# codeslake/RefVSR

Hardware: AMD Instinct MI355X
Metric: 4x SR frames/sec (270p->1080p, RefVSR_small_L1) (higher is better)
Workload: dtype f16; 1 GPU; config_RefVSR_small_L1 4x SR, 270x480 -> 1080x1920, frame_num=5, steady-state sliding window, n=1 (BASELINE configs[1]); synthetic clip seed 0, seeded random weights 1234; frames_per_rank=20, parallelism=frame-shard x1 (reset-aligned, no collective), window_cache=True, frame_ids=True, pipelined_calls=True, frames_per_call=4, headline_mode=frame groups, pipe_layout=pfm, full=False

## Files before the change

include/refvsr_hip.h:

```cpp
#ifndef REFVSR_HIP_H
#define REFVSR_HIP_H

#include <stddef.h>
#include <stdint.h>

#ifdef __cplusplus
extern "C" {
#endif

#define REFVSR_ABI_VERSION 15

int refvsr_abi_version(void);
int refvsr_max_maps(void);
const char* refvsr_last_error(void);
int refvsr_init(void);

int refvsr_num_cus(void);
int refvsr_stream_create_cu_range(int first_cu, int n_cus, void** stream);
int refvsr_stream_set_cu_budget(void* stream, int n_cus);
int refvsr_stream_destroy(void* stream);

enum { REFVSR_OUT_NHWC16 = 0, REFVSR_OUT_NHWC16_SHUFFLE2 = 1, REFVSR_OUT_PLANAR32 = 2 };

typedef struct RefvsrConv {
// ... 67 lines not shown
                     float* out, void* stream);
int refvsr_conv_hr_last(const void* src, int h, int w, const void* blob, float act_slope, const float* base_lr, int bh, int bw,
                        float* out, void* stream);
enum { REFVSR_RESULT_F32 = 0, REFVSR_RESULT_F16 = 1, REFVSR_RESULT_U8 = 2 };
int refvsr_conv_last_fmt(const void* src, int c, int h, int w, const void* blob, const float* base_lr, int bh, int bw,
                         void* out, int out_fmt, void* stream);
int refvsr_conv_hr_last_fmt(const void* src, int h, int w, const void* blob, float act_slope, const float* base_lr, int bh, int bw,
                            void* out, int out_fmt, void* stream);
int refvsr_convert_result(const float* src, size_t n, int out_fmt, void* out, void* stream);

int refvsr_conf_alpha(const float* conf_a, const float* conf_b, int h, int w, int up, const float* w0, const float* b0,
                      float slope0, const void* blob, int cout, float slope1, void* alpha, float* conf_max, void* stream);
int refvsr_conf_alpha_batch(const float* const* conf_a, const float* const* conf_b, int batch, int h, int w, int up, const float* w0,
                            const float* b0, float slope0, const void* blob, int cout, float slope1, void* const* alpha,
                            float* const* conf_max, void* stream);
int refvsr_conv32_supported(int c0, int c1);
int refvsr_conv32_blob_bytes(int c0, int c1);
int refvsr_conv32(const void* src0, int c0, const void* src1, int c1, int h, int w, const void* blob, float act_slope,
                  const void* mul, const void* res, float post_slope, void* out, void* stream);
int refvsr_conv48_supported(int c0, int c1);
int refvsr_conv48_blob_bytes(int c0, int c1);
int refvsr_conv48(const void* src0, int c0, const void* src1, int c1, int h, int w, const void* blob, float act_slope,
                  const void* mul, const void* res, float post_slope, void* out, void* stream);
int refvsr_conv_shuffle2_supported(int c);
int refvsr_conv_shuffle2_blob_bytes(int c);
int refvsr_conv_shuffle2(const void* src, int c, int h, int w, const void* blobs, float act_slope, void* out, void* stream);
int refvsr_conv_shuffle2_batch(const void* const* src, int batch, int c, int h, int w, const void* blobs, float act_slope,
                               void* const* out, void* stream);
int refvsr_conv24_f16w_blob_bytes(int c0, int c1);
int refvsr_conv32_f16w_blob_bytes(int c0, int c1);
int refvsr_conv_shuffle2_f16w_blob_bytes(int c);
int refvsr_conv24_f16w(const void* src0, int c0, const void* src1, int c1, int h, int w, const void* blob, float act_slope,
                       const void* mul, const void* res, float post_slope, void* out, void* stream);
int refvsr_conv24_batch_f16w(const void* const* src0, int c0, const void* const* src1, int c1, int batch, int h, int w, const void* blob,
                             float act_slope, const void* const* mul, const void* const* res, float post_slope, void* const* out,
                             void* stream);
int refvsr_conv32_f16w(const void* src0, int c0, const void* src1, int c1, int h, int w, const void* blob, float act_slope,
                       const void* mul, const void* res, float post_slope, void* out, void* stream);
int refvsr_conv_shuffle2_f16w(const void* src, int c, int h, int w, const void* blobs, float act_slope, void* out, void* stream);
int refvsr_conv_shuffle2_batch_f16w(const void* const* src, int batch, int c, int h, int w, const void* blobs, float act_slope,
                                    void* const* out, void* stream);
int refvsr_conf_alpha_f16w(const float* conf_a, const float* conf_b, int h, int w, int up, const float* w0, const float* b0,
                           float slope0, const void* blob, int cout, float slope1, void* alpha, float* conf_max, void* stream);
int refvsr_conf_alpha_batch_f16w(const float* const* conf_a, const float* const* conf_b, int batch, int h, int w, int up, const float* w0,
                                 const float* b0, float slope0, const void* blob, int cout, float slope1, void* const* alpha,
                                 float* const* conf_max, void* stream);
int refvsr_set_probe(void* buf, int iter);

int refvsr_conv_direct_f32(const float* src, int cin, int h, int w,
                           const float* wgt, const float* bias, int cout, int ksize, int stride, int pad,
                           float act_slope, void* out, int out_nhwc16, int out_c, void* stream);
int refvsr_conv1x1_f32(const float* src, int cin, int h, int w, const float* wgt, const float* bias, float act_slope,
                       float* out, void* stream);

int refvsr_pack_nhwc16(const float* src, int c, int h, int w, void* dst, int cs, void* stream);
int refvsr_pack_nhwc32(const float* src, int c, int h, int w, float* dst, int cs, void* stream);
int refvsr_unpack_nhwc16(const void* src, int h, int w, int cs, int c, float* dst, void* stream);

enum { REFVSR_RS_BICUBIC = 0, REFVSR_RS_BILINEAR = 1, REFVSR_RS_BILINEAR_AC = 2, REFVSR_RS_NEAREST = 3 };
int refvsr_resize(const float* src, int c, int h, int w, void* dst, int oh, int ow, int mode,
                  float src_scale_y, float src_scale_x, const float* mean, const float* std,
                  const float* chan_mul, int clamp01, int out_nhwc16, int out_c, void* stream);
int refvsr_avgpool2(const float* src, int c, int h, int w, float* dst, void* stream);
int refvsr_maxpool2(const float* src, int c, int h, int w, float* dst, void* stream);
int refvsr_avgpool_pyramid(const float* src, int c, int h, int w, float* const* dst, void* stream);
int refvsr_frame_prep(const float* lr, int h, int w, const float* ref, int hr, int wr, const float* wgt, const float* bias,
                      void* lr8, void* ref8, float* lr_n, float* ref_n, void* stream);
int refvsr_buffers_equal(const void* const* a, const void* const* b, int n_pairs, size_t n_bytes,
                         int32_t* flags, void* stream);
int refvsr_bytes_equal(const void* const* a, const void* const* b, int n_pairs, size_t n_bytes,
                       int32_t* flags, void* stream);
int refvsr_max2(const float* a, const float* b, float* out, size_t n, void* stream);

#define REFVSR_INGEST_MAX_FRAMES 16
enum { REFVSR_INGEST_PLANAR = 0, REFVSR_INGEST_HWC = 1 };
int refvsr_ingest_u8(const void* const* src, float* const* dst, int nframes, int h, int w, int layout, void* stream);
int refvsr_ingest_table(float* out);
int refvsr_ingest_max_frames(void);

#define REFVSR_SCORE_MAX_FRAMES 16
size_t refvsr_score_workspace_bytes(int nframes, int h, int w);
int refvsr_score_max_frames(void);
int refvsr_score_frames(const void* const* out, int out_fmt, const void* const* gt, int gt_fmt, int gt_layout, int nframes, int h, int w,
                        int win, void* workspace, size_t workspace_bytes, double* scores, void* stream);

int refvsr_score_frames_down(const void* const* out, int out_fmt, const void* const* gt, int gt_fmt, int gt_layout, int nframes, int h,
                             int w, int down, int win, void* workspace, size_t workspace_bytes, double* scores, void* stream);

#define REFVSR_SCORE_MAX_RECTS 8
size_t refvsr_score_regions_workspace_bytes(int nframes, int h, int w, int nrects);
int refvsr_score_max_rects(void);
int refvsr_score_regions(const void* const* out, int out_fmt, const void* const* gt, int gt_fmt, int gt_layout, int nframes, int h, int w,
                         const int* rects, int nrects, void* workspace, size_t workspace_bytes, double* sums, void* stream);

#define REFVSR_COLORMAP_MAX_MAPS 16
int refvsr_conf_colormap(const void* const* maps, int n, int h, int w, void* const* rgb, void* ws, size_t ws_bytes, void* stream);
size_t refvsr_conf_colormap_workspace_bytes(int n, int h, int w);
int refvsr_colormap_table(unsigned char* out768);

int refvsr_warp_nhwc16(const void* x, int hin, int win, int cs, const float* flow, int hf, int wf,
                       void* out, void* stream);
int refvsr_warp_nhwc16_up2(const void* x, int hin, int win, int cs, const float* flow_lr, int hl, int wl,
                           void* out, void* stream);
int refvsr_warp_planar(const float* x, int c, int hin, int win, const float* flow, int hf, int wf,
                       float* out, void* stream);
int refvsr_warp_nhwc16_batch(const void* const* x, int batch, int hin, int win, int cs, const float* const* flow, int hf, int wf,
// ... 48 lines not shown
```

refvsr_amd/engine.py:

```python
import collections
import itertools
import os

import torch

from . import ops
from .config import resolve_weight_precision
from .knobs import env_flag
from .packing import pack_conv
from .weights import VGG_MEAN, VGG_STD, round16

_uid = itertools.count()


def _timed_event(stream):
    e = torch.cuda.Event(enable_timing=True)
    e.record(stream)
    return e


def _flow_pairs(fr, restart):
    t = len(fr)
    ctr = t // 2
    need = [(fr[i], fr[i + 1]) for i in range(ctr, t - 1)] + [(fr[ctr + 1], fr[ctr])]
# ... 124 lines not shown
        reslist('feat_decoder_BWFW', 4)
        for br in ('backward_resblocks', 'forward_resblocks'):
            cin = sd['Network.' + br + '.main.0.weight'].shape[1]
            if cin == C + 3:
                mf(br + '.main.0', [3, C])
            else:
                assert cin == 2 * C + 3
                mf(br + '.main.0', [3, C, C])
                cw = self.conv[br + '.main.0']
                cw.cpads = [cw.cpads[0] + cw.cpads[1], cw.cpads[2]]
            for i in range(self.nb):
                mf('%s.main.2.%d.conv1' % (br, i), [C])
                mf('%s.main.2.%d.conv2' % (br, i), [C])
        mf('fusion_UP', [C, C])
        mf('upsample1.upsample_conv', [C], shuffle=True)
        if config.scale == 4:
            mf('upsample2.upsample_conv', [C], shuffle=True)
        mf('conv_hr', [C])
        mf('conv_last', [C])


class Engine(object):

    def __init__(self, config, weights):
        if config.scale not in (2, 4):
            raise NotImplementedError('SR scale must be 2 or 4 (configs/config_RefVSR_*.py: "SR scale (2 | 4)")')
        self.cfg = config
        self.W = weights
        self.C = config.mid_channels
        self.nb = config.num_blocks
        self.ks = config.matching_ksize
        self.hd = bool(config.flag_HD_in)
        self.vgg7 = self.hd or config.scale != 4
        self.cache = bool(getattr(config, 'cache_windows', True))
        self.match_row_splits = 1
        self.match_margin = float(getattr(config, 'match_exact_margin', ops.MATCH_EXACT_MARGIN))
        self.chain_calls = bool(getattr(config, 'chain_calls', not env_flag('REFVSR_NO_CHAIN_CALLS')))
        self.fuse_resblocks = (bool(getattr(config, 'fuse_resblocks', True)) and ops.resblock_fits(self.C)
                               and not env_flag('REFVSR_NO_FUSE'))
        self.rb24 = not env_flag('REFVSR_NO_RB24')
        self.rb48 = (bool(getattr(config, 'fuse_resblocks', True)) and not env_flag('REFVSR_NO_FUSE')
                     and not env_flag('REFVSR_NO_RB48'))
        self.rb48_max_pixels = int(os.environ.get('REFVSR_RB48_MAX_PIXELS', str(540 * 960)))
        self.rb48_multimap = not env_flag('REFVSR_NO_RB48_MULTIMAP')
        self.spynet_mt1_pixels = int(os.environ.get('REFVSR_SPYNET_MT1_PIXELS', str(72 * 120)))
        self.bw_head_blocks = min(self.nb, max(-1, int(getattr(config, 'bw_head_blocks', None) if getattr(config, 'bw_head_blocks', None) is not None
                                                         else os.environ.get('REFVSR_BW_HEAD_BLOCKS', '12'))))
        self.warp_up2 = not env_flag('REFVSR_NO_WARP_UP2')
        self.fuse_head = not env_flag('REFVSR_NO_FUSE_HEAD')
        self.fuse_tail = self.fuse_head and (env_flag('REFVSR_FUSE_TAIL') or bool(getattr(config, 'fuse_tail', False)))
        self.fuse_conf = not env_flag('REFVSR_NO_FUSE_CONF')
        self.map1x1 = not env_flag('REFVSR_NO_MAP1X1')
        self.legacy_prep = env_flag('REFVSR_LEGACY_PREP')
        self.last_flagged = None
        self.spynet_batch = not env_flag('REFVSR_NO_SPYNET_BATCH')
        self.overlap = bool(getattr(config, 'overlap_streams', True)) and not env_flag('REFVSR_NO_OVERLAP')
        self._side = None
        self.pipelined = bool(getattr(config, 'pipelined', False))
        self._zero_maps = {}
        self.result_dtype = str(getattr(config, 'result_dtype', None) or 'float32').replace('torch.', '')
        ops.result_format(self.result_dtype)
        self._pipe = None
        self._layout_default = None
        self.pipe_depth = max(1, int(getattr(config, 'pipe_depth', None) or os.environ.get('REFVSR_PIPE_DEPTH') or 3))
        self._inflight = collections.deque()
        self.stream_events = None
        self.kernel_events = None
        self.chain_events = None
        self.reset_state()

    def reset_state(self):
        self.fw_feat = None
        self.fw_flow = None
        self.fw_feat_up = None
        self.fw_conf = None
        self.frame_itr_num = 0
        self.max_frame_itr_num = self.cfg.reset_branch
        self.prev_window = []
        self.flow_cache = {}
        self.id_cache = {}
        self.ctx_pinned = {}
        self.ctx_strict = False
        self._fw_up_wait = None

    def set_pipelined(self, on=True):
        self.pipelined = bool(on)

    def export_state(self):
        if self.fw_feat is None:
            return None
        self._await_fw_up(self.fw_feat_up)
        st = dict(feat=ops.unpack_nhwc16(self.fw_feat, self.C), flow=self.fw_flow, feat_up=ops.unpack_nhwc16(self.fw_feat_up, self.C),
                  conf=self.fw_conf, frame_itr_num=self.frame_itr_num)
        kf = getattr(self, 'keyframe_idx', None)
        if kf is not None:
            st['keyframe_idx'] = [int(k) for k in kf]
        return st

    def import_state(self, st):
        cs = (self.C + 7) // 8 * 8
        self.fw_feat = ops.pack_nhwc16(st['feat'].contiguous(), cs)
        self.fw_flow = st['flow'].contiguous()
        self.fw_feat_up = ops.pack_nhwc16(st['feat_up'].contiguous(), cs)
        self.fw_conf = st['conf'].contiguous()
        self.frame_itr_num = int(st['frame_itr_num'])
        if st.get('keyframe_idx') is not None and hasattr(self, 'keyframe_idx'):
# ... 334 lines not shown
                x = ops.conv(cw if cw is not None else self.cw(p + '%d.conv' % j), x, act=0.0, batch=B)
            flow = ops.conv(self.cw(p + '4.conv'), x, planar_out=True, res_planar=fup, batch=B)
        h_up, w_up = flow.shape[2:]
        cm = [float(w) / float(w_up), float(h) / float(h_up)]
        outs = [ops.resize(flow[b0:b0 + 2].reshape(-1, h_up, w_up), (h, w), ops.RS_BILINEAR, chan_mul=cm * min(2, B - b0))
                for b0 in range(0, B, 2)]
        out = outs[0].view(-1, 2, h, w) if len(outs) == 1 else torch.cat([o_.view(-1, 2, h, w) for o_ in outs], 0)
        ev = None
        if share:
            ev = torch.cuda.Event()
            ev.record()
            for st in share:
                out.record_stream(st)
        for i, (a, b) in enumerate(todo):
            self.flow_cache[(a.uid, b.uid)] = (out[i], ev)

    def frame_prep(self, fr):
        if self.hd or self.legacy_prep:
            return None
        return ops.frame_prep(fr.lr, fr.ref, *self.W.raw['feature_match.sub_mean'])

    def feature_match(self, fr, prep=None):
        R = self.W.raw
        h, w = fr.lr.shape[1:]

        fe = 'feature_match.feature_extract.'

        def extract(x):
            x = ops.conv(self.cw(fe + '0'), x, act=0.0)
            if not self.vgg7:
                x = ops.conv(self.cw(fe + '2'), x, act=0.0)
                if self.map1x1:
                    return ops.conv1x1_f32(x, *R[fe + 'map64.0'], act=0.2)
                return ops.conv(self.cw(fe + 'map64.0'), x, act=0.2, planar_out=True)
            x = ops.conv(self.cw(fe + '2'), x, act=0.0, planar_out=True)
            x = ops.pack_nhwc32(ops.maxpool2(x))
            x = ops.conv(self.cw(fe + '5'), x, act=0.0)
            if self.map1x1:
                return ops.conv1x1_f32(x, *R[fe + 'map128.0'], act=0.2)
            return ops.conv(self.cw(fe + 'map128.0'), x, act=0.2, planar_out=True)
        if prep is None:
            prep = self.frame_prep(fr)
        if prep is not None:
            lr_n, ref_n = prep[2], prep[3]
        else:
            lr_n = ops.conv_direct(fr.lr, *R['feature_match.sub_mean'])
            ref_n = ops.conv_direct(fr.ref, *R['feature_match.sub_mean'])
            if self.hd:
                f = 1.0 / (self.cfg.scale // 2)
                oh, ow = int(h * f), int(w * f)
                lr_n = ops.resize(lr_n, (oh, ow), ops.RS_NEAREST, (1.0 / f, 1.0 / f))
                ref_n = ops.resize(ref_n, (oh, ow), ops.RS_NEAREST, (1.0 / f, 1.0 / f))
            lr_n, ref_n = ops.pack_nhwc32(lr_n, 4), ops.pack_nhwc32(ops.avgpool2(ref_n), 4)
        lr_f = extract(lr_n)
        ref_f = extract(ref_n)
        ops.set_match_patches_kernel(0 if self.legacy_prep else 1)
        if self.legacy_prep:
            lr_rows, inv_lr, lr_lo = ops.match_patches(lr_f, ops.hip.MATCH_COLBLOCK, want_lo=True)
        else:
            (lr_rows, inv_lr), lr_lo = ops.match_patches(lr_f, ops.hip.MATCH_COLBLOCK), None
        ref_rows, inv_ref, ref_lo = ops.match_patches(ref_f, ops.hip.MATCH_ROWCHUNK, want_lo=True)
        n_lr = lr_f.shape[1] * lr_f.shape[2]
        n_ref = ref_f.shape[1] * ref_f.shape[2]
        if self.kernel_events is not None:
            e0, e1 = torch.cuda.Event(enable_timing=True), torch.cuda.Event(enable_timing=True)
            e0.record()
        cand, cand_val = ops.match_top2(ref_rows, n_ref, lr_rows, n_lr, self.match_row_splits)
        if self.kernel_events is not None:
            e1.record()
            self.kernel_events.append((e0, e1))
        conf, idx, self.last_flagged = ops.match_refine(lr_f, ref_f, inv_lr, inv_ref, cand, cand_val, self.match_margin, (lr_rows, lr_lo),
                                                        (ref_rows, ref_lo))
        conf = conf.view(1, lr_f.shape[1], lr_f.shape[2])
        grid = (lr_f.shape[1], lr_f.shape[2])
        if grid[0] != h:
            conf = ops.bicubic_scale(conf, float(h) / grid[0], clamp01=True)
        return conf, idx, grid

    def aligned_conv(self, feats, query, rgb8, prefix, ks):
        def enc(z8):
            e = ops.conv(self.cw(prefix + '.conv1.0'), z8, act=0.2)
            t = ops.conv(self.cw(prefix + '.conv1.2.conv1'), e, act=0.2)
            return ops.conv(self.cw(prefix + '.conv1.2.conv2'), t, res=e, post=0.2)
        q = enc(ops.bicubic_scale(query, 2, clamp01=False, nhwc16_out=True))
        r = enc(rgb8)
        a = ops.conv(self.cw(prefix + '.p_conv.0'), r, q, stride=ks, act=0.2)
        t = ops.conv(self.cw(prefix + '.p_conv.2.conv1'), a, act=0.2)
        a = ops.conv(self.cw(prefix + '.p_conv.2.conv2'), t, res=a, post=0.2)
        affine = ops.conv(self.cw(prefix + '.p_conv.4'), a, planar_out=True, add_const=1.0, clamp=(-3.0, 3.0))
        return ops.aligned_sample(feats, affine, ks)

    def _ref_encoders(self, fr, ref8=None):
        if ref8 is None:
            ref8 = ops.pack_nhwc16(fr.ref, 8)
        x = ops.conv(self.cw('ref_encoder1.0.0'), ref8, act=0.2)
        x = ops.conv(self.cw('ref_encoder1.1.0'), x, act=0.2)
        ref_feat = self.res_list(x, 'res1', 4)
        x = ops.conv(self.cw('ref_encoder2.0.0'), ref_feat, stride=2, act=0.2)
        x = ops.conv(self.cw('ref_encoder2.1.0'), x, act=0.2)
        return ref_feat, self.res_list(x, 'res2', 4)

    def prepare_frame(self, fr):
        if fr.conf is not None:
            return
        if self.ctx_strict:
            raise RuntimeError('a window needs a per-frame context that was neither prepared ahead nor imported (strict mode)')
        h, w = fr.lr.shape[1:]
        prep = self.frame_prep(fr)
# ... 797 lines not shown
```

refvsr_amd/hip.py:

```python
import ctypes as C
import os

_HERE = os.path.dirname(os.path.abspath(__file__))
LIB_PATH = os.path.join(_HERE, 'librefvsr_hip.so')

OUT_NHWC16, OUT_NHWC16_SHUFFLE2, OUT_PLANAR32 = 0, 1, 2
RS_BICUBIC, RS_BILINEAR, RS_BILINEAR_AC, RS_NEAREST = 0, 1, 2, 3
RESULT_F32, RESULT_F16, RESULT_U8 = 0, 1, 2
INGEST_PLANAR, INGEST_HWC = 0, 1
MATCH_KP, MATCH_ROWCHUNK, MATCH_COLBLOCK = 152, 256, 512
ABI_VERSION = 15
MAX_MAPS = 4
INGEST_MAX_FRAMES = 16
SCORE_MAX_FRAMES = 16
SCORE_MAX_RECTS = 8
COLORMAP_MAX_MAPS = 16
RESBLOCK24_BLOB_BYTES = 43264
RESBLOCK24_F16W_BLOB_BYTES = 28928
RESBLOCK48_BLOB_BYTES = 172544


class RefvsrConv(C.Structure):
    _fields_ = [
        ('src0', C.c_void_p), ('c0', C.c_int),
# ... 74 lines not shown
    'refvsr_conv_hr_last_fmt': [_P, _I, _I, _P, _F, _P, _I, _I, _P, _I, _P],
    'refvsr_convert_result': [_P, _Z, _I, _P, _P],
    'refvsr_conf_alpha': [_P, _P, _I, _I, _I, _P, _P, _F, _P, _I, _F, _P, _P, _P],
    'refvsr_spynet_level_input_batch': [_P, _P, _I, _P, _I, _I, _P, _P, _P],
    'refvsr_resblock24_chain_batch': [_P, _I, _I, _I, _I, _P, _Z, _F, _P, _P, _P, _P],
    'refvsr_resblock48_chain_batch': [_P, _I, _I, _I, _I, _P, _Z, _F, _P, _P, _P, _P],
    'refvsr_conv24_batch': [_P, _I, _P, _I, _I, _I, _I, _P, _F, _P, _P, _F, _P, _P],
    'refvsr_conv_shuffle2_batch': [_P, _I, _I, _I, _I, _P, _F, _P, _P],
    'refvsr_conf_alpha_batch': [_P, _P, _I, _I, _I, _I, _P, _P, _F, _P, _I, _F, _P, _P, _P],
    'refvsr_warp_nhwc16_batch': [_P, _I, _I, _I, _I, _P, _I, _I, _P, _P],
    'refvsr_warp_nhwc16_up2_batch': [_P, _I, _I, _I, _I, _P, _I, _I, _P, _P],
    'refvsr_warp_planar_batch': [_P, _I, _I, _I, _I, _P, _I, _I, _P, _P],
    'refvsr_match_patches': [_P, _I, _I, _P, _P, _P, _P],
    'refvsr_match_top2': [_P, _I, _P, _I, _I, _P, _P, _P],
    'refvsr_match_refine': [_P, _I, _I, _P, _I, _I, _P, _P, _P, _P, _I, _F, _P, _P, _P, _P],
    'refvsr_match_exact': [_P, _I, _I, _P, _I, _I, _P, _P, _P, _P, _P, _P, _P, _P, _P, _P, _P],
    'refvsr_match_naive': [_P, _I, _I, _P, _I, _I, _P, _P, _P],
    'refvsr_block_gather_nhwc16': [_P, _I, _I, _I, _P, _I, _I, _I, _P, _P],
    'refvsr_block_gather_rgb': [_P, _I, _I, _P, _I, _I, _I, _P, _P, _P],
    'refvsr_aligned_sample': [_P, _I, _I, _I, _I, _P, _P, _P],
    'refvsr_dcn_sample': [_P, _I, _I, _I, _P, _I, _P, _P],
    'refvsr_tsa_weight': [_P, _P, _P, _I, _I, _I, _P, _P],
    'refvsr_pool3s2_nhwc16': [_P, _I, _I, _I, _P, _I, _I, _I, _P],
    'refvsr_up2_bilinear_nhwc16': [_P, _I, _I, _I, _F, _P, _P],
    'refvsr_tsa_blend': [_P, _P, _P, _Z, _P, _P],
    'refvsr_resblock24_f16w_blob_bytes': [],
    'refvsr_conv24_f16w_blob_bytes': [_I, _I],
    'refvsr_conv32_f16w_blob_bytes': [_I, _I],
    'refvsr_conv_shuffle2_f16w_blob_bytes': [_I],
    'refvsr_resblock24_chain_f16w': [_P, _I, _I, _I, _P, _Z, _F, _P, _P, _P, _P],
    'refvsr_resblock24_chain_batch_f16w': [_P, _I, _I, _I, _I, _P, _Z, _F, _P, _P, _P, _P],
    'refvsr_conv24_f16w': [_P, _I, _P, _I, _I, _I, _P, _F, _P, _P, _F, _P, _P],
    'refvsr_conv24_batch_f16w': [_P, _I, _P, _I, _I, _I, _I, _P, _F, _P, _P, _F, _P, _P],
    'refvsr_conv32_f16w': [_P, _I, _P, _I, _I, _I, _P, _F, _P, _P, _F, _P, _P],
    'refvsr_conv_shuffle2_f16w': [_P, _I, _I, _I, _P, _F, _P, _P],
    'refvsr_conv_shuffle2_batch_f16w': [_P, _I, _I, _I, _I, _P, _F, _P, _P],
    'refvsr_conf_alpha_f16w': [_P, _P, _I, _I, _I, _P, _P, _F, _P, _I, _F, _P, _P, _P],
    'refvsr_conf_alpha_batch_f16w': [_P, _P, _I, _I, _I, _I, _P, _P, _F, _P, _I, _F, _P, _P, _P],
    'refvsr_ingest_u8': [_P, _P, _I, _I, _I, _I, _P],
    'refvsr_ingest_table': [_P],
    'refvsr_ingest_max_frames': [],
    'refvsr_bytes_equal': [_P, _P, _I, _Z, _P, _P],
    'refvsr_score_frames': [_P, _I, _P, _I, _I, _I, _I, _I, _I, _P, _Z, _P, _P],
    'refvsr_score_max_frames': [],
    'refvsr_score_frames_down': [_P, _I, _P, _I, _I, _I, _I, _I, _I, _I, _P, _Z, _P, _P],
    'refvsr_score_regions': [_P, _I, _P, _I, _I, _I, _I, _I, _P, _I, _P, _Z, _P, _P],
    'refvsr_score_max_rects': [],
    'refvsr_set_match_patches_kernel': [_I],
    'refvsr_match_lo_rows': [_P, _I, _I, _P, _P, _P, _P],
    'refvsr_avgpool_pyramid': [_P, _I, _I, _I, _P, _P],
    'refvsr_frame_prep': [_P, _I, _I, _P, _I, _I, _P, _P, _P, _P, _P, _P, _P],
    'refvsr_conf_colormap': [_P, _I, _I, _I, _P, _P, _Z, _P],
    'refvsr_colormap_table': [_P],
}
_SPECIAL = {'refvsr_abi_version': (C.c_int, []), 'refvsr_last_error': (C.c_char_p, []),
            'refvsr_score_workspace_bytes': (C.c_size_t, [_I, _I, _I]),
            'refvsr_score_regions_workspace_bytes': (C.c_size_t, [_I, _I, _I, _I]),
            'refvsr_conf_colormap_workspace_bytes': (C.c_size_t, [_I, _I, _I])}
EXPORTS = tuple(sorted(list(SIGNATURES) + list(_SPECIAL)))

_lib = None


def lib():
    global _lib
    if _lib is None:
        if not os.path.exists(LIB_PATH):
            raise RuntimeError(
                'refvsr_amd: %s not found -- the HIP extension is required (no CPU fallback). '
                'Build it with `make -C refvsr_amd/csrc` or `python -c "import __graft_entry__ as g; g.build()"`.'
                % LIB_PATH)
        h = C.CDLL(LIB_PATH)
        for name, args in SIGNATURES.items():
            fn = getattr(h, name)
            fn.argtypes = args
            fn.restype = C.c_int
        for name, (res, args) in _SPECIAL.items():
            fn = getattr(h, name)
            fn.argtypes = args
            fn.restype = res
        if h.refvsr_abi_version() != ABI_VERSION:
            raise RuntimeError('refvsr_amd: ABI mismatch (library %d, binding %d)' % (h.refvsr_abi_version(), ABI_VERSION))
        if h.refvsr_max_maps() != MAX_MAPS:
            raise RuntimeError('refvsr_amd: REFVSR_MAX_MAPS mismatch (library %d, binding %d)' % (h.refvsr_max_maps(), MAX_MAPS))
        if h.refvsr_ingest_max_frames() != INGEST_MAX_FRAMES:
            raise RuntimeError('refvsr_amd: REFVSR_INGEST_MAX_FRAMES mismatch (library %d, binding %d)'
                               % (h.refvsr_ingest_max_frames(), INGEST_MAX_FRAMES))
        if h.refvsr_score_max_frames() != SCORE_MAX_FRAMES:
            raise RuntimeError('refvsr_amd: REFVSR_SCORE_MAX_FRAMES mismatch (library %d, binding %d)'
                               % (h.refvsr_score_max_frames(), SCORE_MAX_FRAMES))
        if h.refvsr_score_max_rects() != SCORE_MAX_RECTS:
            raise RuntimeError('refvsr_amd: REFVSR_SCORE_MAX_RECTS mismatch (library %d, binding %d)'
                               % (h.refvsr_score_max_rects(), SCORE_MAX_RECTS))
        _lib = h
    return _lib


def check(rc, what):
    if rc != 0:
        msg = lib().refvsr_last_error()
        raise RuntimeError('refvsr_hip.%s failed (rc=%d): %s' % (what, rc, msg.decode() if msg else '?'))
```

refvsr_amd/ops.py:

```python
import ctypes as C
import math
import os

import torch

from . import hip
from .knobs import env_flag
from .hip import (OUT_NHWC16, OUT_NHWC16_SHUFFLE2, OUT_PLANAR32, RS_BICUBIC, RS_BILINEAR,
                  RS_BILINEAR_AC, RS_NEAREST)


_STREAM = None


def _stream():
    if _STREAM is not None:
        return _STREAM
    return C.c_void_p(torch.cuda.current_stream().cuda_stream)


class on_stream(object):

    def __init__(self, stream):
        self.stream = stream
# ... 408 lines not shown
    hip.check(hip.lib().refvsr_convert_result(_ptr(x), x.numel(), fmt, _ptr(out), _stream()), 'convert_result')
    return out


def conv_last(blob, src, base_lr, result_dtype=None):
    _nhwc(src)
    _planar(base_lr, 3)
    h, w, c = src.shape
    bh, bw = base_lr.shape[1:]
    dt, fmt = result_format(result_dtype)
    out = torch.empty((3, h, w), dtype=dt, device=src.device)
    hip.check(hip.lib().refvsr_conv_last_fmt(_ptr(src), c, h, w, _ptr(blob), _ptr(base_lr), bh, bw, _ptr(out), fmt, _stream()), 'conv_last')
    return out


def conv_hr_last(blob, src, base_lr, act=0.1, result_dtype=None):
    _nhwc(src)
    _planar(base_lr, 3)
    h, w, c = src.shape
    assert c == 24 and blob.numel() == hip.RESBLOCK24_BLOB_BYTES
    bh, bw = base_lr.shape[1:]
    dt, fmt = result_format(result_dtype)
    out = torch.empty((3, h, w), dtype=dt, device=src.device)
    hip.check(hip.lib().refvsr_conv_hr_last_fmt(_ptr(src), h, w, _ptr(blob), act, _ptr(base_lr), bh, bw, _ptr(out), fmt, _stream()), 'conv_hr_last')
    return out


def conv_last_ok(c, h, w):
    return bool(hip.lib().refvsr_conv_last_supported(int(c))) and h * w * c * 2 < 2 ** 31


def conf_alpha_ok(cw):
    return cw.blob24 is not None and cw.cpads == [16] and cw.cout in (24, 48) and not cw.shuffle


def pack_nhwc16(x, cs=None):
    _planar(x)
    c, h, w = x.shape
    cs = cs or (c + 7) // 8 * 8
    out = torch.empty((h, w, cs), dtype=torch.float16, device=x.device)
    hip.check(hip.lib().refvsr_pack_nhwc16(_ptr(x), c, h, w, _ptr(out), cs, _stream()), 'pack_nhwc16')
    return out


def conv1x1_f32(x, w, b, act=0.2):
    assert x.is_cuda and x.dtype == torch.float32 and x.dim() == 3 and x.is_contiguous()
    h, w_, cin = x.shape
    assert tuple(w.shape) == (16, cin) and w.dtype == torch.float32 and w.is_contiguous() and tuple(b.shape) == (16,)
    out = torch.empty((16, h, w_), dtype=torch.float32, device=x.device)
    hip.check(hip.lib().refvsr_conv1x1_f32(_ptr(x), cin, h, w_, _ptr(w), _ptr(b), float(act), _ptr(out), _stream()), 'conv1x1_f32')
    return out


def pack_nhwc32(x, cs=None):
    _planar(x)
    c, h, w = x.shape
    cs = cs or (c + 3) // 4 * 4
    out = torch.empty((h, w, cs), dtype=torch.float32, device=x.device)
    hip.check(hip.lib().refvsr_pack_nhwc32(_ptr(x), c, h, w, _ptr(out), cs, _stream()), 'pack_nhwc32')
    return out


def unpack_nhwc16(x, c=None):
    _nhwc(x)
    h, w, cs = x.shape
    c = c or cs
    out = torch.empty((c, h, w), dtype=torch.float32, device=x.device)
    hip.check(hip.lib().refvsr_unpack_nhwc16(_ptr(x), h, w, cs, c, _ptr(out), _stream()), 'unpack_nhwc16')
    return out


def resize(x, out_hw, mode, src_scale=None, mean=None, std=None, chan_mul=None, clamp01=False, nhwc16_out=False):
    _planar(x)
    c, h, w = x.shape
    oh, ow = out_hw
    if src_scale is None:
        src_scale = (float(h) / float(oh), float(w) / float(ow))
    if nhwc16_out:
        out = torch.empty((oh, ow, 8), dtype=torch.float16, device=x.device)
    else:
        out = torch.empty((c, oh, ow), dtype=torch.float32, device=x.device)
    hip.check(hip.lib().refvsr_resize(_ptr(x), c, h, w, _ptr(out), oh, ow, mode, src_scale[0], src_scale[1],
                                      _farr(mean), _farr(std), _farr(chan_mul), int(clamp01), int(nhwc16_out),
                                      8 if nhwc16_out else 0, _stream()), 'resize')
    return out


def bicubic_scale(x, factor, clamp01=True, nhwc16_out=False):
    c, h, w = x.shape
    oh, ow = int(math.floor(h * factor)), int(math.floor(w * factor))
    s = 1.0 / factor
    return resize(x, (oh, ow), RS_BICUBIC, (s, s), clamp01=clamp01, nhwc16_out=nhwc16_out)


def flow_up2(flow):
    c, h, w = flow.shape
    return resize(flow, (2 * h, 2 * w), RS_BILINEAR_AC, (0.0, 0.0), chan_mul=[2.0] * c)


def avgpool2(x):
    _planar(x)
    c, h, w = x.shape
    out = torch.empty((c, h // 2, w // 2), dtype=torch.float32, device=x.device)
    hip.check(hip.lib().refvsr_avgpool2(_ptr(x), c, h, w, _ptr(out), _stream()), 'avgpool2')
    return out

# ... 594 lines not shown
```

Baseline: 233.3 frames/s.

## Fuse VGG feature-match head (conv0, conv2, 1x1 map) into one multi-map kernel

Adds a single HIP kernel that runs the feature-match VGG head in one pass: first 3x3 conv (3->64), second 3x3 conv (64->64) via f32 MFMA with a ring-buffered LDS weight pipeline, and the 64->16 1x1 map. It covers both LR and reference maps in one launch and is used by default when the 1x1 map path is active. This removes the intermediate 64-channel feature maps in global memory and several kernel launches. In exchange it adds heavy LDS use per block (low occupancy) and recomputes a halo for conv0 in each tile.

Result: no change. 235.3 frames/s (median of 6 runs) (+0.9%).

```diff
diff --git a/include/refvsr_hip.h b/include/refvsr_hip.h
--- a/include/refvsr_hip.h
+++ b/include/refvsr_hip.h
@@ -143,6 +143,9 @@
                            float act_slope, void* out, int out_nhwc16, int out_c, void* stream);
 int refvsr_conv1x1_f32(const float* src, int cin, int h, int w, const float* wgt, const float* bias, float act_slope,
                        float* out, void* stream);
+int refvsr_vgg_head(const void* const* src, const int* h, const int* w, int n, const void* wpack0, const float* bias0,
+                    const void* wpack2, const float* bias2, const float* wmap, const float* bmap, float map_slope,
+                    void* const* out, void* stream);
 
 int refvsr_pack_nhwc16(const float* src, int c, int h, int w, void* dst, int cs, void* stream);
 int refvsr_pack_nhwc32(const float* src, int c, int h, int w, float* dst, int cs, void* stream);
diff --git a/refvsr_amd/csrc/vgg_head.hip b/refvsr_amd/csrc/vgg_head.hip
--- /dev/null
+++ b/refvsr_amd/csrc/vgg_head.hip
@@ -0,0 +1,325 @@
+#include "common.h"
+
+#define VH_NW 8
+#define VH_TH 8
+#define VH_TW 32
+#define VH_XH (VH_TH + 4)
+#define VH_XW (VH_TW + 4)
+#define VH_FH (VH_TH + 2)
+#define VH_FW (VH_TW + 2)
+#define VH_FPIX (VH_FH * VH_FW)
+#define VH_PS 17
+#define VH_S0 3
+#define VH_S2 36
+#define VH_CH 4
+#define VH_NCHUNK (VH_S2 / VH_CH)
+#define VH_NS 3
+#define VH_SLOT (VH_CH * 4 * 1024)
+#define VH_PPW (VH_CH * 4 / VH_NW)
+#define VH_YS 65
+
+#define VH_OFF_TAB2 0
+#define VH_OFF_TAB0 (VH_S2 * 16)
+#define VH_OFF_RING 640
+#define VH_OFF_X (VH_OFF_RING + VH_NS * VH_SLOT)
+#define VH_OFF_F (VH_OFF_X + VH_XH * VH_XW * 16)
+#define VH_LDS (VH_OFF_F + VH_FPIX * VH_PS * 16)
+
+static_assert(VH_OFF_TAB0 + VH_S0 * 16 <= VH_OFF_RING, "tables");
+static_assert(VH_S2 % VH_CH == 0 && VH_PPW * VH_NW == VH_CH * 4 && VH_CH == 4, "the ring loop is unrolled for 4 full K-steps per chunk");
+static_assert(VH_TH * VH_TW * VH_YS * 4 <= VH_FPIX * VH_PS * 16 && 64 * 16 * 4 <= VH_XH * VH_XW * 16, "epilogue regions");
+static_assert(VH_LDS <= 160 * 1024, "LDS");
+
+struct VHArgs {
+    const unsigned char* src[REFVSR_MAX_MAPS];
+    float* out[REFVSR_MAX_MAPS];
+    int h[REFVSR_MAX_MAPS], w[REFVSR_MAX_MAPS], tiles_x[REFVSR_MAX_MAPS];
+    int t_end[REFVSR_MAX_MAPS];
+    int n;
+    const unsigned char* w0; const float* b0;
+    const unsigned char* w2; const float* b2;
+    const float* wm; const float* bm;
+    float slope;
+};
+
+__global__ __launch_bounds__(VH_NW * 64) void vgg_head_kernel(VHArgs p) {
+    extern __shared__ __attribute__((aligned(16))) unsigned char smem[];
+    int* tab2 = reinterpret_cast<int*>(smem + VH_OFF_TAB2);
+    int* tab0 = reinterpret_cast<int*>(smem + VH_OFF_TAB0);
+    unsigned char* ring = smem + VH_OFF_RING;
+    unsigned char* xt = smem + VH_OFF_X;
+    unsigned char* ft = smem + VH_OFF_F;
+
+    int tl = blockIdx.x;
+    const unsigned char* src = p.src[0];
+    float* out = p.out[0];
+    int h = p.h[0], w = p.w[0], tiles_x = p.tiles_x[0], t0 = 0;
+#pragma unroll
+    for (int m = 1; m < REFVSR_MAX_MAPS; ++m)
+        if (m < p.n && tl >= p.t_end[m - 1]) { src = p.src[m]; out = p.out[m]; h = p.h[m]; w = p.w[m]; tiles_x = p.tiles_x[m]; t0 = p.t_end[m - 1]; }
+    tl -= t0;
+    asm volatile("" :: "s"(src), "s"(out), "s"(h), "s"(w), "s"(tiles_x), "s"(tl), "s"(p.w0), "s"(p.b0), "s"(p.w2), "s"(p.b2),
+                 "s"(p.wm), "s"(p.bm), "s"(p.slope));
+    const int tyi = tl / tiles_x;
+    const int ty0 = tyi * VH_TH;
+    const int tx0 = (tl - tyi * tiles_x) * VH_TW;
+
+    const int tid = threadIdx.x;
+    const int lane = tid & 63;
+    const int wave = tid >> 6;
+    const int q = lane >> 4;
+    const int lp = rv_pix16(lane & 15);
+
+    const int wv = __builtin_amdgcn_readfirstlane(wave);
+    const unsigned char* gw = p.w2 + lane * 16;
+    auto issue = [&](const int c, const int slot) {
+#pragma unroll
+        for (int j = 0; j < VH_PPW; ++j) {
+            const int pc = wv + j * VH_NW;
+            const int s = c * VH_CH + (pc >> 2), m = pc & 3;
+            __builtin_amdgcn_global_load_lds((const __attribute__((address_space(1))) void*)(gw + (((m >> 1) * VH_S2 + s) * 2 + (m & 1)) * 1024),
+                                             (__attribute__((address_space(3))) void*)(ring + slot * VH_SLOT + pc * 1024), 16, 0, 0);
+        }
+    };
+    int slot_w = 0;
+    for (int c = 0; c < VH_NS - 1; ++c) { issue(c, slot_w); ++slot_w; }
+
+    if (tid < VH_S2 * 4) {
+        const int tap = tid >> 4, cg = tid & 15;
+        const int ty = tap / 3, tx = tap - ty * 3;
+        tab2[rv_kslot(ty, tx, cg, 3, 16)] = ((ty * VH_FW + tx) * VH_PS + cg) * 16;
+    } else if (tid < VH_S2 * 4 + VH_S0 * 4) {
+        const int g = tid - VH_S2 * 4;
+        if (g < 9) {
+            const int ty = g / 3, tx = g - ty * 3;
+            tab0[rv_kslot(ty, tx, 0, 3, 1)] = (ty * VH_XW + tx) * 16;
+        } else {
+            tab0[rv_kpad_slot(g - 9, 3, 1)] = 16;
+        }
+    }
+    if (tid < VH_XH * VH_XW) {
+        const int r = tid / VH_XW, c = tid - r * VH_XW;
+        const int iy = ty0 - 2 + r, ix = tx0 - 2 + c;
+        const bool ok = (unsigned)iy < (unsigned)h && (unsigned)ix < (unsigned)w;
+        const size_t pix = (size_t)min(max(iy, 0), h - 1) * w + min(max(ix, 0), w - 1);
+        uint4 v = *reinterpret_cast<const uint4*>(src + pix * 16);
+        const unsigned keep = ok ? 0xffffffffu : 0u;
+        v.x &= keep; v.y &= keep; v.z &= keep; v.w &= keep;
+        *reinterpret_cast<uint4*>(xt + tid * 16) = v;
+    }
+    uint4 a0w[VH_S0][4];
+    float4 b0r[4];
+#pragma unroll
+    for (int s = 0; s < VH_S0; ++s)
+#pragma unroll
+        for (int m = 0; m < 4; ++m)
+            a0w[s][m] = *reinterpret_cast<const uint4*>(p.w0 + ((((m >> 1) * VH_S0 + s) * 2 + (m & 1)) * 64 + lane) * 16);
+#pragma unroll
+    for (int m = 0; m < 4; ++m) b0r[m] = *reinterpret_cast<const float4*>(p.b0 + m * 16 + q * 4);
+    __syncthreads();
+
+    for (int g = wave; g * 16 < VH_FPIX; g += VH_NW) {
+        const int pp = g * 16 + lp;
+        const int pc = min(pp, VH_FPIX - 1);
+        const int r = pc / VH_FW, c = pc - r * VH_FW;
+        const unsigned char* xb = xt + (r * VH_XW + c) * 16;
+        f32x4 acc0[4];
+#pragma unroll
+        for (int m = 0; m < 4; ++m) acc0[m] = (f32x4){0.f, 0.f, 0.f, 0.f};
+#pragma unroll
+        for (int s = 0; s < VH_S0; ++s) {
+            const f32x4 bv = *reinterpret_cast<const f32x4*>(xb + tab0[s * 4 + q]);
+#pragma unroll
+            for (int m = 0; m < 4; ++m) {
+                const f32x4 av = *reinterpret_cast<const f32x4*>(&a0w[s][m]);
+#pragma unroll
+                for (int j = 0; j < 4; ++j) acc0[m] = __builtin_amdgcn_mfma_f32_16x16x4f32(av[j], bv[j], acc0[m], 0, 0, 0);
+            }
+        }
+        const int iy = ty0 - 1 + r, ix = tx0 - 1 + c;
+        const bool inside = (unsigned)iy < (unsigned)h && (unsigned)ix < (unsigned)w;
+        if (pp < VH_FPIX) {
+#pragma unroll
+            for (int m = 0; m < 4; ++m) {
+                float y[4];
+                const float4 bv = b0r[m];
+                y[0] = acc0[m][0] + bv.x; y[1] = acc0[m][1] + bv.y; y[2] = acc0[m][2] + bv.z; y[3] = acc0[m][3] + bv.w;
+#pragma unroll
+                for (int i = 0; i < 4; ++i) y[i] = inside ? rv_lrelu(y[i], 0.0f) : 0.0f;
+                *reinterpret_cast<f32x4*>(ft + (pp * VH_PS + m * 4 + q) * 16) = (f32x4){y[0], y[1], y[2], y[3]};
+            }
+        }
+    }
+
+    f32x4 acc[4][2];
+#pragma unroll
+    for (int m = 0; m < 4; ++m)
+#pragma unroll
+        for (int t = 0; t < 2; ++t) acc[m][t] = (f32x4){0.f, 0.f, 0.f, 0.f};
+    {
+        const unsigned lds_tab = (unsigned)(size_t)(__attribute__((address_space(3))) unsigned char*)reinterpret_cast<unsigned char*>(tab2);
+        const unsigned lds_ring = (unsigned)(size_t)(__attribute__((address_space(3))) unsigned char*)ring;
+        const unsigned lds_ft = (unsigned)(size_t)(__attribute__((address_space(3))) unsigned char*)ft;
+        unsigned pbaddr[2];
+#pragma unroll
+        for (int t = 0; t < 2; ++t) pbaddr[t] = lds_ft + (unsigned)(((wave * VH_FW + t * 16 + lp) * VH_PS) * 16);
+        typedef unsigned u32x4 __attribute__((ext_vector_type(4)));
+        auto tie = [](uint4& r) {
+            u32x4 t = {r.x, r.y, r.z, r.w};
+            asm volatile("" : "+v"(t));
+            r = make_uint4(t[0], t[1], t[2], t[3]);
+        };
+        auto wait_set = [&](uint4 (&a)[4], uint4 (&b)[2]) {
+            asm volatile("s_waitcnt lgkmcnt(6)" ::: "memory");
+#pragma unroll
+            for (int i = 0; i < 4; ++i) tie(a[i]);
+#pragma unroll
+            for (int t = 0; t < 2; ++t) tie(b[t]);
+        };
+        auto mfma_step = [&](const uint4 (&a)[4], const uint4 (&b)[2]) {
+#pragma unroll
+            for (int t = 0; t < 2; ++t) {
+                const f32x4 bv = *reinterpret_cast<const f32x4*>(&b[t]);
+#pragma unroll
+                for (int m = 0; m < 4; ++m) {
+                    const f32x4 av = *reinterpret_cast<const f32x4*>(&a[m]);
+#pragma unroll
+                    for (int j = 0; j < 4; ++j) acc[m][t] = __builtin_amdgcn_mfma_f32_16x16x4f32(av[j], bv[j], acc[m][t], 0, 0, 0);
+                }
+            }
+        };
+        auto compute_chunk = [&](const unsigned wslot, const int s0) {
+            unsigned toff[VH_CH];
+#pragma unroll
+            for (int j = 0; j < VH_CH; ++j)
+                asm volatile("ds_read_b32 %0, %1" : "=v"(toff[j]) : "v"(lds_tab + (unsigned)(((s0 + j) * 4 + q) * 4)));
+            asm volatile("s_waitcnt lgkmcnt(0)" ::: "memory");
+#pragma unroll
+            for (int j = 0; j < VH_CH; ++j) asm volatile("" : "+v"(toff[j]));
+            const unsigned wa = wslot + (unsigned)lane * 16;
+            auto load_set = [&](const int j, uint4 (&a)[4], uint4 (&b)[2]) {
+                const unsigned wj = wa + (unsigned)j * 4096;
+#define VH_LDA(I) { u32x4 v; asm volatile("ds_read_b128 %0, %1 offset:%2" : "=v"(v) : "v"(wj), "n"((I) * 1024)); a[I] = make_uint4(v[0], v[1], v[2], v[3]); }
+                VH_LDA(0) VH_LDA(1) VH_LDA(2) VH_LDA(3)
+#undef VH_LDA
+#pragma unroll
+                for (int t = 0; t < 2; ++t) {
+                    u32x4 v;
+                    asm volatile("ds_read_b128 %0, %1" : "=v"(v) : "v"(pbaddr[t] + toff[j]));
+                    b[t] = make_uint4(v[0], v[1], v[2], v[3]);
+                }
+            };
+            uint4 a0[4], b0[2], a1[4], b1[2];
+            load_set(0, a0, b0);
+            load_set(1, a1, b1);
+            wait_set(a0, b0);
+            __builtin_amdgcn_sched_barrier(0);
+            mfma_step(a0, b0);
+            load_set(2, a0, b0);
+            wait_set(a1, b1);
+            __builtin_amdgcn_sched_barrier(0);
+            mfma_step(a1, b1);
+            load_set(3, a1, b1);
+            wait_set(a0, b0);
+            __builtin_amdgcn_sched_barrier(0);
+            mfma_step(a0, b0);
+            asm volatile("s_waitcnt lgkmcnt(0)" ::: "memory");
+#pragma unroll
+            for (int i = 0; i < 4; ++i) tie(a1[i]);
+#pragma unroll
+            for (int t = 0; t < 2; ++t) tie(b1[t]);
+            __builtin_amdgcn_sched_barrier(0);
+            mfma_step(a1, b1);
+        };
+        int slot_r = 0;
+        for (int c = 0; c < VH_NCHUNK; ++c) {
+            if (c == VH_NCHUNK - 1) asm volatile("s_waitcnt vmcnt(0)" ::: "memory");
+            else asm volatile("s_waitcnt vmcnt(%0)" :: "n"(VH_PPW) : "memory");
+            asm volatile("s_waitcnt lgkmcnt(0)" ::: "memory");
+            __builtin_amdgcn_s_barrier();
+            asm volatile("" ::: "memory");
+            if (c + VH_NS - 1 < VH_NCHUNK) { issue(c + VH_NS - 1, slot_w); slot_w = slot_w + 1 == VH_NS ? 0 : slot_w + 1; }
+            compute_chunk(lds_ring + (unsigned)slot_r * VH_SLOT, c * VH_CH);
+            slot_r = slot_r + 1 == VH_NS ? 0 : slot_r + 1;
+        }
+    }
+
+    __syncthreads();
+    float* ys = reinterpret_cast<float*>(ft);
+    float* ws = reinterpret_cast<float*>(xt);
+#pragma unroll
+    for (int m = 0; m < 4; ++m) {
+        const float4 bv = *reinterpret_cast<const float4*>(p.b2 + m * 16 + q * 4);
+#pragma unroll
+        for (int t = 0; t < 2; ++t) {
+            float y[4];
+            y[0] = acc[m][t][0] + bv.x; y[1] = acc[m][t][1] + bv.y; y[2] = acc[m][t][2] + bv.z; y[3] = acc[m][t][3] + bv.w;
+            float* d = ys + (wave * VH_TW + t * 16 + lp) * VH_YS + m * 16 + q * 4;
+#pragma unroll
+            for (int i = 0; i < 4; ++i) d[i] = rv_lrelu(y[i], 0.0f);
+        }
+    }
+    for (int i = tid; i < 64 * 16; i += VH_NW * 64) ws[i] = p.wm[(i & 15) * 64 + (i >> 4)];
+    __syncthreads();
+
+    const size_t npix = (size_t)h * w;
+#pragma unroll
+    for (int k = 0; k < 2; ++k) {
+        const int item = tid + k * (VH_NW * 64);
+        const int px = item & (VH_TH * VH_TW - 1), og = item >> 8;
+        const float* xp = ys + px * VH_YS;
+        float a0 = 0.f, a1 = 0.f, a2 = 0.f, a3 = 0.f;
+        for (int c = 0; c < 64; ++c) {
+            const float x = xp[c];
+            const float4 w4 = *reinterpret_cast<const float4*>(ws + c * 16 + og * 4);
+            a0 = fmaf(x, w4.x, a0); a1 = fmaf(x, w4.y, a1); a2 = fmaf(x, w4.z, a2); a3 = fmaf(x, w4.w, a3);
+        }
+        const int oy = ty0 + (px >> 5), ox = tx0 + (px & 31);
+        if (oy < h && ox < w) {
+            float* o = out + (size_t)(og * 4) * npix + (size_t)oy * w + ox;
+            o[0] = rv_lrelu(a0 + p.bm[og * 4 + 0], p.slope);
+            o[npix] = rv_lrelu(a1 + p.bm[og * 4 + 1], p.slope);
+            o[2 * npix] = rv_lrelu(a2 + p.bm[og * 4 + 2], p.slope);
+            o[3 * npix] = rv_lrelu(a3 + p.bm[og * 4 + 3], p.slope);
+        }
+    }
+}
+
+extern "C" int refvsr_vgg_head(const void* const* src, const int* h, const int* w, int n, const void* wpack0, const float* bias0,
+                               const void* wpack2, const float* bias2, const float* wmap, const float* bmap, float map_slope,
+                               void* const* out, void* stream) {
+    RV_CHECK(n >= 1 && n <= REFVSR_MAX_MAPS, "vgg_head: 1..%d maps per launch (got %d)", REFVSR_MAX_MAPS, n);
+    RV_CHECK(src && h && w && out, "vgg_head: null map table");
+    RV_CHECK(wpack0 && bias0 && wpack2 && bias2 && wmap && bmap, "vgg_head: null weights / bias");
+    RV_CHECK(((uintptr_t)wpack0 & 15) == 0 && ((uintptr_t)wpack2 & 15) == 0 && ((uintptr_t)bias0 & 15) == 0 && ((uintptr_t)bias2 & 15) == 0,
+             "vgg_head: weight blobs and biases must be 16-byte aligned");
+    RV_CHECK(map_slope >= 0.f && map_slope <= 1.f, "vgg_head: activation slope must lie in [0, 1]");
+    VHArgs a;
+    memset(&a, 0, sizeof(a));
+    long long tiles = 0;
+    for (int m = 0; m < n; ++m) {
+        RV_CHECK(src[m] && out[m], "vgg_head: null map pointer (map %d)", m);
+        RV_CHECK(((uintptr_t)src[m] & 15) == 0 && ((uintptr_t)out[m] & 3) == 0, "vgg_head: map %d is not aligned", m);
+        RV_CHECK(h[m] > 0 && w[m] > 0 && (long long)h[m] * w[m] < (1ll << 27), "vgg_head: bad size of map %d (%d x %d)", m, h[m], w[m]);
+        for (int k = 0; k < n; ++k) RV_CHECK(src[m] != out[k] && (k == m || out[k] != out[m]), "vgg_head: buffers must be distinct");
+        a.src[m] = (const unsigned char*)src[m]; a.out[m] = (float*)out[m];
+        a.h[m] = h[m]; a.w[m] = w[m];
+        a.tiles_x[m] = rv_cdiv(w[m], VH_TW);
+        tiles += (long long)a.tiles_x[m] * rv_cdiv(h[m], VH_TH);
+        a.t_end[m] = (int)tiles;
+    }
+    RV_CHECK(tiles < (1ll << 30), "vgg_head: too many tiles");
+    RV_CHECK(refvsr_init() == 0, "init failed");
+    a.n = n;
+    a.w0 = (const unsigned char*)wpack0; a.b0 = bias0; a.w2 = (const unsigned char*)wpack2; a.b2 = bias2;
+    a.wm = wmap; a.bm = bmap; a.slope = map_slope;
+    static bool attr_done[RV_MAX_DEVICES] = {};
+    const int dev = rv_device();
+    if (!attr_done[dev]) {
+        RV_HIP(hipFuncSetAttribute(reinterpret_cast<const void*>(&vgg_head_kernel), hipFuncAttributeMaxDynamicSharedMemorySize, 160 * 1024));
+        attr_done[dev] = true;
+    }
+    hipLaunchKernelGGL(vgg_head_kernel, dim3((unsigned)tiles), dim3(VH_NW * 64), VH_LDS, (hipStream_t)stream, a);
+    RV_LAUNCH_CHECK();
+    return 0;
+}
diff --git a/refvsr_amd/engine.py b/refvsr_amd/engine.py
--- a/refvsr_amd/engine.py
+++ b/refvsr_amd/engine.py
@@ -200,6 +200,7 @@
         self.fuse_conf = not env_flag('REFVSR_NO_FUSE_CONF')
         self.map1x1 = not env_flag('REFVSR_NO_MAP1X1')
         self.legacy_prep = env_flag('REFVSR_LEGACY_PREP')
+        self.vgg_head = not self.vgg7 and self.map1x1 and not env_flag('REFVSR_NO_VGG_HEAD')
         self.last_flagged = None
         self.spynet_batch = not env_flag('REFVSR_NO_SPYNET_BATCH')
         self.overlap = bool(getattr(config, 'overlap_streams', True)) and not env_flag('REFVSR_NO_OVERLAP')
@@ -640,8 +641,11 @@
                 lr_n = ops.resize(lr_n, (oh, ow), ops.RS_NEAREST, (1.0 / f, 1.0 / f))
                 ref_n = ops.resize(ref_n, (oh, ow), ops.RS_NEAREST, (1.0 / f, 1.0 / f))
             lr_n, ref_n = ops.pack_nhwc32(lr_n, 4), ops.pack_nhwc32(ops.avgpool2(ref_n), 4)
-        lr_f = extract(lr_n)
-        ref_f = extract(ref_n)
+        if self.vgg_head:
+            lr_f, ref_f = ops.vgg_head([lr_n, ref_n], self.cw(fe + '0'), self.cw(fe + '2'), R[fe + 'map64.0'], act=0.2)
+        else:
+            lr_f = extract(lr_n)
+            ref_f = extract(ref_n)
         ops.set_match_patches_kernel(0 if self.legacy_prep else 1)
         if self.legacy_prep:
             lr_rows, inv_lr, lr_lo = ops.match_patches(lr_f, ops.hip.MATCH_COLBLOCK, want_lo=True)
diff --git a/refvsr_amd/hip.py b/refvsr_amd/hip.py
--- a/refvsr_amd/hip.py
+++ b/refvsr_amd/hip.py
@@ -150,6 +150,7 @@
     'refvsr_frame_prep': [_P, _I, _I, _P, _I, _I, _P, _P, _P, _P, _P, _P, _P],
     'refvsr_conf_colormap': [_P, _I, _I, _I, _P, _P, _Z, _P],
     'refvsr_colormap_table': [_P],
+    'refvsr_vgg_head': [_P, _P, _P, _I, _P, _P, _P, _P, _P, _P, _F, _P, _P],
 }
 _SPECIAL = {'refvsr_abi_version': (C.c_int, []), 'refvsr_last_error': (C.c_char_p, []),
             'refvsr_score_workspace_bytes': (C.c_size_t, [_I, _I, _I]),
diff --git a/refvsr_amd/ops.py b/refvsr_amd/ops.py
--- a/refvsr_amd/ops.py
+++ b/refvsr_amd/ops.py
@@ -484,6 +484,25 @@
     return out
 
 
+def vgg_head(maps, w0, w2, w_map, act=0.2):
+    n = len(maps)
+    assert 1 <= n <= hip.MAX_MAPS, 'vgg_head takes 1..%d maps (got %d)' % (hip.MAX_MAPS, n)
+    for cw, cin, ks in ((w0, 4, 3), (w2, 64, 36)):
+        assert cw.f32 and cw.mt == 2 and cw.cout == 64 and cw.ksize == 3 and list(cw.cpads) == [cin] and cw.ksteps == ks, \
+            'vgg_head needs the f32-packed 3x3 convs 3 -> 64 and 64 -> 64 (mt = 2)'
+    wm, bm = w_map
+    assert tuple(wm.shape) == (16, 64) and wm.dtype == torch.float32 and wm.is_contiguous() and tuple(bm.shape) == (16,) and bm.dtype == torch.float32
+    for x in maps:
+        _nhwc(x, True)
+        assert x.shape[2] == 4, 'vgg_head input maps are packed fp32 [h,w,4]'
+    outs = [torch.empty((16, x.shape[0], x.shape[1]), dtype=torch.float32, device=x.device) for x in maps]
+    hs = (C.c_int * n)(*[x.shape[0] for x in maps])
+    ws = (C.c_int * n)(*[x.shape[1] for x in maps])
+    hip.check(hip.lib().refvsr_vgg_head(_parr(maps), hs, ws, n, _ptr(w0.wpack), _ptr(w0.bias), _ptr(w2.wpack), _ptr(w2.bias), _ptr(wm), _ptr(bm),
+                                        float(act), _parr(outs), _stream()), 'vgg_head')
+    return outs
+
+
 def pack_nhwc32(x, cs=None):
     _planar(x)
     c, h, w = x.shape
```
